# Youngju-Na/UFORecon

Hardware: AMD Instinct MI355X
Metric: rays/s (per-ray volume-rendering path, 64+64 hierarchical samples, DTU-shaped 3-view 512x640) (higher is better)
Workload: dtype f32; 1 GPU; configs[1]: full 512x640 frame = 327680 rays, 3 source views, 64+64 samples, rays sharded by row tiles over 1 GPU(s), depth/RGB tiles all-gathered; rays_per_frame=327680, chunk_rays=4096, side_streams=3

## Files before the change

### uforecon_amd/csrc/gather.hip

```cpp
#include "ufr_device.h"
#include "ufr_internal.h"
#include "volume_sample.h"

namespace ufr {

__device__ __forceinline__ f32x4 lerp_tap4_buf(__amdgpu_buffer_rsrc_t r, unsigned base, int stride_bytes, const Tap2& t, unsigned c4) {
  f32x4 v[4];
#pragma unroll
  for (int k = 0; k < 4; ++k)
    v[k] = buf_ld4(r, t.o[k] >= 0 ? base + __umul24((unsigned)t.o[k], (unsigned)stride_bytes) + c4 : kBufOut);
  f32x4 acc;
#pragma unroll
  for (int e = 0; e < 4; ++e) {
    float a = mul_rn(v[0][e], t.w[0]);
    a = fmaf(v[1][e], t.w[1], a);
    a = fmaf(v[2][e], t.w[2], a);
    acc[e] = fmaf(v[3][e], t.w[3], a);
  }
  return acc;
}

typedef int i32x4 __attribute__((ext_vector_type(4)));

__device__ __forceinline__ void put_tap(float* dst, const Tap2& t) {
  *reinterpret_cast<i32x4*>(dst) = i32x4{t.o[0], t.o[1], t.o[2], t.o[3]};
  *reinterpret_cast<f32x4*>(dst + 4) = f32x4{t.w[0], t.w[1], t.w[2], t.w[3]};
}
__device__ __forceinline__ Tap2 get_tap(const float* src) {
  const i32x4 o = *reinterpret_cast<const i32x4*>(src);
  const f32x4 w = *reinterpret_cast<const f32x4*>(src + 4);
  Tap2 t;
#pragma unroll
  for (int k = 0; k < 4; ++k) { t.o[k] = o[k]; t.w[k] = w[k]; }
  return t;
}

__device__ __forceinline__ void presim_block(const PreSim& ps, const float* sim, int sim_stride, float* out, int out_stride,
                                             int lane) {
  const int g = lane >> 4, j = lane & 15;
  f32x4 h1[4][2], h2[4][2], o[4];
  float x0[4][2];
#pragma unroll
  for (int u = 0; u < 4; ++u) {
    const float* sq = sim + (16 * u + j) * sim_stride;
    x0[u][0] = sq[g];
    x0[u][1] = sq[4 + g];
  }
  {
    float a1[2][2];
#pragma unroll
    for (int to = 0; to < 2; ++to) {
#pragma unroll
      for (int s = 0; s < 2; ++s) a1[to][s] = ps.w0[(16 * to + j) * 8 + 4 * s + g];
      const f32x4 b1 = ld4(ps.b0 + 16 * to + 4 * g);
#pragma unroll
      for (int u = 0; u < 4; ++u) h1[u][to] = b1;
    }
#pragma unroll
    for (int s = 0; s < 2; ++s)
#pragma unroll
      for (int to = 0; to < 2; ++to)
#pragma unroll
        for (int u = 0; u < 4; ++u) h1[u][to] = mfma16(a1[to][s], x0[u][s], h1[u][to]);
  }
  {
    float a2[2][2][4];
#pragma unroll
    for (int to = 0; to < 2; ++to) {
#pragma unroll
      for (int ti = 0; ti < 2; ++ti)
#pragma unroll
        for (int r = 0; r < 4; ++r) a2[to][ti][r] = ps.w2[(16 * to + j) * 32 + 16 * ti + 4 * g + r];
      const f32x4 b2 = ld4(ps.b2 + 16 * to + 4 * g);
#pragma unroll
      for (int u = 0; u < 4; ++u) h2[u][to] = b2;
    }
#pragma unroll
    for (int ti = 0; ti < 2; ++ti)
#pragma unroll
      for (int r = 0; r < 4; ++r)
#pragma unroll
        for (int to = 0; to < 2; ++to)
#pragma unroll
          for (int u = 0; u < 4; ++u) h2[u][to] = mfma16(a2[to][ti][r], fmaxf(h1[u][ti][r], 0.f), h2[u][to]);
  }
  {
    float a3[2][4];
#pragma unroll
    for (int to = 0; to < 2; ++to)
#pragma unroll
      for (int r = 0; r < 4; ++r) a3[to][r] = ps.w4[j * 32 + 16 * to + 4 * g + r];
    const f32x4 b3 = ld4(ps.b4 + 4 * g);
#pragma unroll
    for (int u = 0; u < 4; ++u) o[u] = b3;
#pragma unroll
    for (int ti = 0; ti < 2; ++ti)
#pragma unroll
      for (int r = 0; r < 4; ++r)
#pragma unroll
        for (int u = 0; u < 4; ++u) o[u] = mfma16(a3[ti][r], fmaxf(h2[u][ti][r], 0.f), o[u]);
  }
#pragma unroll
  for (int u = 0; u < 4; ++u) st4(out + (16 * u + j) * out_stride + 24 + 4 * g, o[u]);
}

template <int NVT>
__global__ void __launch_bounds__(64 * NVT) gather_kernel(FrameDev f, PreSim ps, const float* __restrict__ ray_o,
                                                      int o_stride, const float* __restrict__ ray_d,
                                                      const float* __restrict__ zval, int P, int SN,
                                                      float* __restrict__ x_tokens, float* __restrict__ x_point,
                                                      float* __restrict__ rgb_out,
                                                      float* __restrict__ dir_out, float* __restrict__ sim8_out,
                                                      float* __restrict__ vol24_out, float* __restrict__ xy_out,
                                                      float* __restrict__ maskz_out,
                                                      const float* __restrict__ vol24_in,
                                                      const float* __restrict__ sim8_in) {
  extern __shared__ __attribute__((aligned(16))) float smem[];
  constexpr int NV = NVT;
  constexpr int npair = NV * (NV - 1) / 2;
  float* sh_sim = smem;
  float* sh_tapF = sh_sim + 64 * npair * 8;
  float* sh_tapM = sh_tapF + NV * 64 * 8;
  float* sh_vol = sh_tapF;
  constexpr int sim_slot = npair * 8;
  constexpr bool out_in_sim = sim_slot >= 48;
  constexpr int region2 = 2 * NV * 64 * 8 > 64 * (NV - 1) * 25 ? 2 * NV * 64 * 8 : 64 * (NV - 1) * 25;
  float* sh_out = out_in_sim ? sh_sim + 8 : sh_tapF + region2;
  constexpr int out_stride = out_in_sim ? sim_slot : 40;

  const int v = threadIdx.x >> 6, p = threadIdx.x & 63;
  const int vu = __builtin_amdgcn_readfirstlane(v);
  const int nb8 = (int)(gridDim.x / 8) * 8;
  const int blk = (int)blockIdx.x < nb8 ? (int)(blockIdx.x % 8) * (nb8 / 8) + (int)(blockIdx.x / 8) : (int)blockIdx.x;
  const int pidx = blk * 64 + p;
  const bool active = pidx < P;
  const int pc = active ? pidx : P - 1;
  const int ray = pc / SN;

  const float zz = zval[pc];
  const float* o = ray_o + (size_t)ray * o_stride;
  const float px = mul_add_unfused(zz, ray_d[3 * ray + 0], o[0]);
  const float py = mul_add_unfused(zz, ray_d[3 * ray + 1], o[1]);
  const float pz = mul_add_unfused(zz, ray_d[3 * ray + 2], o[2]);

  const float* M = f.pose[v];
  float qx = fmaf(M[2], pz, fmaf(M[1], py, mul_rn(M[0], px))) + M[3];
  float qy = fmaf(M[6], pz, fmaf(M[5], py, mul_rn(M[4], px))) + M[7];
  float qz = fmaf(M[10], pz, fmaf(M[9], py, mul_rn(M[8], px))) + M[11];
  const float mask_z = qz > 0.f ? 1.f : 0.f;
  const float x = qx / qz, y = qy / qz;
  if (active && xy_out) {
    xy_out[((size_t)v * P + pidx) * 2 + 0] = x;
    xy_out[((size_t)v * P + pidx) * 2 + 1] = y;
  }
  if (active && maskz_out) maskz_out[(size_t)v * P + pidx] = mask_z;

  const int row_cols = x_point ? kViewCols : UFR_TOKEN_DIM, pe_col = x_point ? 32 : 72;
  float* xrow = x_tokens + ((size_t)pc * NV + v) * row_cols;

  {
    put_tap(sh_tapF + (v * 64 + p) * 8, taps_zeros(unnorm2d_nac(x, f.w), unnorm2d_nac(y, f.h), f.w, f.h));
    put_tap(sh_tapM + (v * 64 + p) * 8, taps_border(unnorm2d_ac(x, f.w), unnorm2d_ac(y, f.h), f.w, f.h));
    Tap2 tf = taps_zeros(unnorm2d_nac(x, f.W), unnorm2d_nac(y, f.H), f.W, f.H);
    const unsigned img_px = (unsigned)(f.H * f.W);
    f32x4 c4 = lerp_tap4_buf(buf_rsrc(f.rgb + (size_t)vu * img_px * 4, img_px * 16u), 0u, 16, tf, 0u);
    const float inb = (x <= 1.f && x >= -1.f && y <= 1.f && y >= -1.f) ? 1.f : 0.f;
    c4[3] = inb * mask_z;
    if (active) st4(rgb_out + ((size_t)pidx * NV + v) * 4, c4);
    float dv[4];
    const __amdgpu_buffer_rsrc_t rdepth = buf_rsrc(f.depth + (size_t)vu * img_px, img_px * 4u);
#pragma unroll
    for (int k = 0; k < 4; ++k) dv[k] = buf_ld1(rdepth, tf.o[k] >= 0 ? (unsigned)tf.o[k] * 4u : kBufOut);
    const float dm = fmaf(dv[3], tf.w[3], fmaf(dv[2], tf.w[2], fmaf(dv[1], tf.w[1], mul_rn(dv[0], tf.w[0]))));
    const float* R = f.w2c_z[v];
    float zc = fmaf(R[2], pz, fmaf(R[1], py, mul_rn(R[0], px))) + R[3];
    float delta = dm - zc;
    float pe[8];
#pragma unroll
    for (int k = 0; k < 4; ++k) {
      const float fr = 3.14159274101257324f * (float)(1 << k);
      pe[2 * k] = sinf(mul_rn(delta, fr));
      pe[2 * k + 1] = sinf(fmaf(delta, fr, 1.57079637050628662f));
    }
    if (active) {
      st4(xrow + pe_col, f32x4{pe[0], pe[1], pe[2], pe[3]});
      st4(xrow + pe_col + 4, f32x4{pe[4], pe[5], pe[6], pe[7]});
    }
    float ax = px - f.ref_pos[0], ay = py - f.ref_pos[1], az = pz - f.ref_pos[2];
    float bx = px - f.cam_pos[v][0], by = py - f.cam_pos[v][1], bz = pz - f.cam_pos[v][2];
    const float ra = __builtin_amdgcn_rcpf(sqrtf(ax * ax + ay * ay + az * az));
    const float rb = __builtin_amdgcn_rcpf(sqrtf(bx * bx + by * by + bz * bz));
    if (active) st4(dir_out + ((size_t)pidx * NV + v) * 4, f32x4{ax * ra - bx * rb, ay * ra - by * rb, az * ra - bz * rb, 0.f});
  }

  __syncthreads();

  const int c8 = threadIdx.x & 7, grp = threadIdx.x >> 3;
  constexpr int n_grp = 64 * NV / 8;
  const unsigned map_px = (unsigned)(f.h * f.w);
  const __amdgpu_buffer_rsrc_t rfeat = buf_rsrc(f.feat, (unsigned)NV * map_px * 128u);
  const __amdgpu_buffer_rsrc_t rmatch = buf_rsrc(f.match, (unsigned)NV * map_px * (unsigned)f.match_ch * 4u);
  for (int item = grp; item < 64 * NV; item += n_grp) {
    const int ip = item / NV, iv = item - ip * NV;
    const int ipidx = blk * 64 + ip;
    if (ipidx < P) {
      const Tap2 t = get_tap(sh_tapF + (iv * 64 + ip) * 8);
      st4(x_tokens + ((size_t)ipidx * NV + iv) * row_cols + 4 * c8,
          lerp_tap4_buf(rfeat, (unsigned)iv * map_px * 128u, 128, t, 16u * c8));
    }
  }
  if (!sim8_in)
  for (int item = grp; item < 64 * npair; item += n_grp) {
    const int ip = item / npair, q = item - ip * npair;
    int a = 0, rem = q;
    while (rem >= NV - 1 - a) { rem -= NV - 1 - a; ++a; }
    const int b = a + rem;
    const int va = a, ca = b, vb = b + 1, cb = a;
    const Tap2 ta = get_tap(sh_tapM + (va * 64 + ip) * 8), tb = get_tap(sh_tapM + (vb * 64 + ip) * 8);
    const unsigned mrow = (unsigned)f.match_ch * 4u;
    f32x4 fa = lerp_tap4_buf(rmatch, (unsigned)va * map_px * mrow + 128u * ca, (int)mrow, ta, 16u * c8);
    f32x4 fb = lerp_tap4_buf(rmatch, (unsigned)vb * map_px * mrow + 128u * cb, (int)mrow, tb, 16u * c8);
    float na = fmaxf(sqrtf(fa[0] * fa[0] + fa[1] * fa[1] + fa[2] * fa[2] + fa[3] * fa[3]), 1e-8f);
    float nb = fmaxf(sqrtf(fb[0] * fb[0] + fb[1] * fb[1] + fb[2] * fb[2] + fb[3] * fb[3]), 1e-8f);
    const float ra = __builtin_amdgcn_rcpf(na), rb = __builtin_amdgcn_rcpf(nb);
    sh_sim[(ip * npair + q) * 8 + c8] = (fa[0] * ra) * (fb[0] * rb) + (fa[1] * ra) * (fb[1] * rb) +
                                        (fa[2] * ra) * (fb[2] * rb) + (fa[3] * ra) * (fb[3] * rb);
  }
  __syncthreads();

  float own[25];
  if (vol24_in) {
#pragma unroll
    for (int c = 0; c < 25; ++c) own[c] = 0.f;
  } else {
    const float zn = ((qz - f.vol_near) / (f.vol_far - f.vol_near)) * 2.f - 1.f;
    float fl[24], wl = 0.f;
#pragma unroll
    for (int s = 0; s < UFR_NUM_STAGES; ++s) {
      float fs[8], ws;
      const float* vol = f.vol[s];
      const unsigned vox = (unsigned)(f.vD[s] * f.vH[s] * f.vW[s]);
      sample_volume_buf(buf_rsrc(vol + (size_t)vu * vox * kVolCh, vox * (unsigned)(kVolCh * 4)), f.vD[s], f.vH[s], f.vW[s], x, y, zn,
                        fs, ws);
#pragma unroll
      for (int c = 0; c < 8; ++c) fl[8 * s + c] = fs[c];
      wl = s == 0 ? ws : wl + ws;
    }
#pragma unroll
    for (int c = 0; c < 24; ++c) own[c] = fl[c] * wl;
    own[24] = wl;
    if (v > 0) {
      float* dst = sh_vol + (p * (NV - 1) + (v - 1)) * 25;
#pragma unroll
      for (int c = 0; c < 25; ++c) dst[c] = own[c];
    }
  }
  __syncthreads();

  if (v == 0) {
    float sim[8];
#pragma unroll
    for (int gi = 0; gi < 8; ++gi) {
      float s = 0.f;
      for (int q = 0; q < npair; ++q) s += sh_sim[(p * npair + q) * 8 + gi];
      sim[gi] = s / (float)npair;
      if (sim8_in) sim[gi] = sim8_in[(size_t)pc * 8 + gi];
    }
    float* ov = sh_out + p * out_stride;
    {
      float Wsum = own[24];
      for (int n = 1; n < NV; ++n) Wsum += sh_vol[(p * (NV - 1) + n - 1) * 25 + 24];
      const float rW = 1.f / (Wsum + 1e-8f);
#pragma unroll
      for (int c = 0; c < 24; ++c) {
        float G = own[c];
        for (int n = 1; n < NV; ++n) G += sh_vol[(p * (NV - 1) + n - 1) * 25 + c];
        ov[c] = G * rW;
        if (vol24_in) ov[c] = vol24_in[(size_t)pc * 24 + c];
      }
    }
    {
      float* mine = sh_sim + p * npair * 8;
      st4(mine, f32x4{sim[0], sim[1], sim[2], sim[3]});
      st4(mine + 4, f32x4{sim[4], sim[5], sim[6], sim[7]});
      __builtin_amdgcn_fence(__ATOMIC_RELEASE, "wavefront");
      __builtin_amdgcn_wave_barrier();
      __builtin_amdgcn_fence(__ATOMIC_ACQUIRE, "wavefront");
      presim_block(ps, sh_sim, sim_slot, sh_out, out_stride, p);
    }
    if (active && sim8_out) {
#pragma unroll
      for (int gi = 0; gi < 8; ++gi) sim8_out[(size_t)pidx * 8 + gi] = sim[gi];
    }
    if (active && vol24_out) {
      for (int c = 0; c < 24; ++c) vol24_out[(size_t)pidx * 24 + c] = ov[c];
    }
  }
  __syncthreads();

  if (active && (!x_point || v == 0)) {
    const float* ov = sh_out + p * out_stride;
    float* dst = x_point ? x_point + (size_t)pidx * kPointCols : xrow + 32;
#pragma unroll
    for (int c = 0; c < 40; c += 4) st4(dst + c, ld4(ov + c));
  }
}

hipError_t launch_gather(const FrameDev& f, const PreSim& ps, const float* ray_o, int o_stride, const float* ray_d,
                         const float* z, int RN, int SN, float* x_tokens, float* x_point, float* rgb, float* dir, float* sim8,
                         float* vol24, float* xy, float* mask_z, const float* vol24_in, const float* sim8_in,
                         hipStream_t s) {
  const int P = RN * SN, NV = f.NV;
  const int npair = NV * (NV - 1) / 2;
  const size_t taps = 2 * (size_t)NV * 64 * 8, volp = (size_t)64 * (NV - 1) * 25, outv = npair * 8 >= 48 ? 0 : 64 * 40;
  size_t lds = sizeof(float) * ((size_t)64 * npair * 8 + (taps > volp ? taps : volp) + outv);
  switch (NV) {
#define UFR_GATHER_CASE(N)                                                                                                   \
    case N:                                                                                                                  \
      hipLaunchKernelGGL(gather_kernel<N>, dim3((P + 63) / 64), dim3(64 * N), lds, s, f, ps, ray_o, o_stride, ray_d, z, P, SN, \
                         x_tokens, x_point, rgb, dir, sim8, vol24, xy, mask_z, vol24_in, sim8_in);                          \
      break;
    UFR_GATHER_CASE(2) UFR_GATHER_CASE(3) UFR_GATHER_CASE(4) UFR_GATHER_CASE(5) UFR_GATHER_CASE(6) UFR_GATHER_CASE(7)
#undef UFR_GATHER_CASE
    default: return hipErrorInvalidValue;
  }
  return hipGetLastError();
}

}
```

Baseline: 2.671 million rays/s.

## Coalesce gather epilogue stores across the block and shrink LDS footprint

Rewrites the gather kernel's epilogue so that x_point/x_tokens, vol24_out and sim8_out are written by all threads of the block in contiguous, coalesced strides from LDS, rather than per-point strided stores from wave 0 only. The output staging buffer now aliases the tap/volume region instead of sitting after it, which reduces LDS per block. A min-waves hint is added to launch_bounds to raise occupancy. It also adds optional cycle-counter phase timing behind a compile flag. The trade-offs are possible register spilling from the occupancy hint and reliance on correct LDS aliasing after the barrier.

New measurement: 2.721 million rays/s, median of 6. 1.9% higher.

```diff
diff --git a/uforecon_amd/csrc/gather.hip b/uforecon_amd/csrc/gather.hip
--- a/uforecon_amd/csrc/gather.hip
+++ b/uforecon_amd/csrc/gather.hip
@@ -1,3 +1,5 @@
+#include <algorithm>
+#include <cstdlib>
 #include "ufr_device.h"
 #include "ufr_internal.h"
 #include "volume_sample.h"
@@ -104,8 +106,22 @@
   for (int u = 0; u < 4; ++u) st4(out + (16 * u + j) * out_stride + 24 + 4 * g, o[u]);
 }
 
+constexpr int kGatherMinW = 5;
+
+#ifdef UFR_PHASE_TIMING
+__device__ unsigned long long g_gather_phase[32];
+#define UFR_G_PHASE(i)                                                                 \
+  {                                                                                    \
+    const unsigned long long t_now = __builtin_readcyclecounter();                     \
+    g_acc[i] = t_now - g_prev;                                                         \
+    g_prev = t_now;                                                                    \
+  }
+#else
+#define UFR_G_PHASE(i)
+#endif
+
 template <int NVT>
-__global__ void __launch_bounds__(64 * NVT) gather_kernel(FrameDev f, PreSim ps, const float* __restrict__ ray_o,
+__global__ void __launch_bounds__(64 * NVT, kGatherMinW) gather_kernel(FrameDev f, PreSim ps, const float* __restrict__ ray_o,
                                                       int o_stride, const float* __restrict__ ray_d,
                                                       const float* __restrict__ zval, int P, int SN,
                                                       float* __restrict__ x_tokens, float* __restrict__ x_point,
@@ -124,9 +140,12 @@
   float* sh_vol = sh_tapF;
   constexpr int sim_slot = npair * 8;
   constexpr bool out_in_sim = sim_slot >= 48;
-  constexpr int region2 = 2 * NV * 64 * 8 > 64 * (NV - 1) * 25 ? 2 * NV * 64 * 8 : 64 * (NV - 1) * 25;
-  float* sh_out = out_in_sim ? sh_sim + 8 : sh_tapF + region2;
+  float* sh_out = out_in_sim ? sh_sim + 8 : sh_tapF;
   constexpr int out_stride = out_in_sim ? sim_slot : 40;
+#ifdef UFR_PHASE_TIMING
+  unsigned long long g_acc[8] = {};
+  unsigned long long g_prev = __builtin_readcyclecounter();
+#endif
 
   const int v = threadIdx.x >> 6, p = threadIdx.x & 63;
   const int vu = __builtin_amdgcn_readfirstlane(v);
@@ -194,6 +213,7 @@
   }
 
   __syncthreads();
+  UFR_G_PHASE(0)
 
   const int c8 = threadIdx.x & 7, grp = threadIdx.x >> 3;
   constexpr int n_grp = 64 * NV / 8;
@@ -227,6 +247,7 @@
                                         (fa[2] * ra) * (fb[2] * rb) + (fa[3] * ra) * (fb[3] * rb);
   }
   __syncthreads();
+  UFR_G_PHASE(1)
 
   float own[25];
   if (vol24_in) {
@@ -256,6 +277,7 @@
     }
   }
   __syncthreads();
+  UFR_G_PHASE(2)
 
   if (v == 0) {
     float sim[8];
@@ -266,7 +288,6 @@
       sim[gi] = s / (float)npair;
       if (sim8_in) sim[gi] = sim8_in[(size_t)pc * 8 + gi];
     }
-    float* ov = sh_out + p * out_stride;
     {
       float Wsum = own[24];
       for (int n = 1; n < NV; ++n) Wsum += sh_vol[(p * (NV - 1) + n - 1) * 25 + 24];
@@ -275,35 +296,55 @@
       for (int c = 0; c < 24; ++c) {
         float G = own[c];
         for (int n = 1; n < NV; ++n) G += sh_vol[(p * (NV - 1) + n - 1) * 25 + c];
-        ov[c] = G * rW;
-        if (vol24_in) ov[c] = vol24_in[(size_t)pc * 24 + c];
+        own[c] = G * rW;
+        if (vol24_in) own[c] = vol24_in[(size_t)pc * 24 + c];
       }
     }
-    {
-      float* mine = sh_sim + p * npair * 8;
-      st4(mine, f32x4{sim[0], sim[1], sim[2], sim[3]});
-      st4(mine + 4, f32x4{sim[4], sim[5], sim[6], sim[7]});
-      __builtin_amdgcn_fence(__ATOMIC_RELEASE, "wavefront");
-      __builtin_amdgcn_wave_barrier();
-      __builtin_amdgcn_fence(__ATOMIC_ACQUIRE, "wavefront");
-      presim_block(ps, sh_sim, sim_slot, sh_out, out_stride, p);
-    }
-    if (active && sim8_out) {
-#pragma unroll
-      for (int gi = 0; gi < 8; ++gi) sim8_out[(size_t)pidx * 8 + gi] = sim[gi];
-    }
-    if (active && vol24_out) {
-      for (int c = 0; c < 24; ++c) vol24_out[(size_t)pidx * 24 + c] = ov[c];
-    }
+    __builtin_amdgcn_fence(__ATOMIC_RELEASE, "wavefront");
+    __builtin_amdgcn_wave_barrier();
+    __builtin_amdgcn_fence(__ATOMIC_ACQUIRE, "wavefront");
+    float* mine = sh_sim + p * sim_slot;
+    st4(mine, f32x4{sim[0], sim[1], sim[2], sim[3]});
+    st4(mine + 4, f32x4{sim[4], sim[5], sim[6], sim[7]});
+    float* ov = sh_out + p * out_stride;
+#pragma unroll
+    for (int c = 0; c < 24; c += 4) st4(ov + c, f32x4{own[c], own[c + 1], own[c + 2], own[c + 3]});
+    UFR_G_PHASE(3)
+    __builtin_amdgcn_fence(__ATOMIC_RELEASE, "wavefront");
+    __builtin_amdgcn_wave_barrier();
+    __builtin_amdgcn_fence(__ATOMIC_ACQUIRE, "wavefront");
+    presim_block(ps, sh_sim, sim_slot, sh_out, out_stride, p);
   }
   __syncthreads();
-
-  if (active && (!x_point || v == 0)) {
-    const float* ov = sh_out + p * out_stride;
-    float* dst = x_point ? x_point + (size_t)pidx * kPointCols : xrow + 32;
-#pragma unroll
-    for (int c = 0; c < 40; c += 4) st4(dst + c, ld4(ov + c));
-  }
+  UFR_G_PHASE(4)
+
+  const int npts = P - blk * 64 < 64 ? P - blk * 64 : 64;
+  if (x_point) {
+    float* dst = x_point + (size_t)blk * 64 * kPointCols;
+    for (int i = threadIdx.x; i < npts * 10; i += 64 * NV) {
+      const int ip = i / 10, c = i - ip * 10;
+      st4(dst + 4 * i, ld4(sh_out + ip * out_stride + 4 * c));
+    }
+  } else {
+    for (int i = threadIdx.x; i < npts * NV * 10; i += 64 * NV) {
+      const int row = i / 10, c = i - row * 10;
+      st4(x_tokens + ((size_t)blk * 64 * NV + row) * UFR_TOKEN_DIM + 32 + 4 * c, ld4(sh_out + (row / NV) * out_stride + 4 * c));
+    }
+  }
+  if (vol24_out)
+    for (int i = threadIdx.x; i < npts * 24; i += 64 * NV) {
+      const int ip = i / 24;
+      vol24_out[(size_t)blk * 64 * 24 + i] = sh_out[ip * out_stride + (i - ip * 24)];
+    }
+  if (sim8_out)
+    for (int i = threadIdx.x; i < npts * 8; i += 64 * NV) sim8_out[(size_t)blk * 64 * 8 + i] = sh_sim[(i >> 3) * sim_slot + (i & 7)];
+  UFR_G_PHASE(5)
+#ifdef UFR_PHASE_TIMING
+  if (threadIdx.x == 0) {
+    for (int i = 0; i < 6; ++i) atomicAdd(&g_gather_phase[i], g_acc[i]);
+    atomicAdd(&g_gather_phase[6], 1ull);
+  }
+#endif
 }
 
 hipError_t launch_gather(const FrameDev& f, const PreSim& ps, const float* ray_o, int o_stride, const float* ray_d,
@@ -313,7 +354,7 @@
   const int P = RN * SN, NV = f.NV;
   const int npair = NV * (NV - 1) / 2;
   const size_t taps = 2 * (size_t)NV * 64 * 8, volp = (size_t)64 * (NV - 1) * 25, outv = npair * 8 >= 48 ? 0 : 64 * 40;
-  size_t lds = sizeof(float) * ((size_t)64 * npair * 8 + (taps > volp ? taps : volp) + outv);
+  size_t lds = sizeof(float) * ((size_t)64 * npair * 8 + std::max(std::max(taps, volp), outv));
   switch (NV) {
 #define UFR_GATHER_CASE(N)                                                                                                   \
     case N:                                                                                                                  \
@@ -328,3 +369,16 @@
 }
 
 }
+
+#ifdef UFR_PHASE_TIMING
+extern "C" int ufr_debug_gather_phases(unsigned long long* out, int n, int reset) {
+  unsigned long long h[32] = {};
+  if (hipMemcpyFromSymbol(h, HIP_SYMBOL(ufr::g_gather_phase), sizeof(h)) != hipSuccess) return -1;
+  for (int i = 0; i < n && i < 32; ++i) out[i] = h[i];
+  if (reset) {
+    unsigned long long z[32] = {};
+    if (hipMemcpyToSymbol(HIP_SYMBOL(ufr::g_gather_phase), z, sizeof(z)) != hipSuccess) return -1;
+  }
+  return 0;
+}
+#endif
```
